# rogeliolopezcamara/prob-matrix-factorization

Measured on AMD Instinct MI355X. Metric: ratings/sec (epoch) Gaussian-MF K=64, higher is better.
Workload: dtype f32; 1 GPU; gaussian_mf_cavi_bias K=64, 1Mx100k synthetic, 50M ratings; n_items=100000, ratings_total=50000000, n_factors=64, ratings_on_rank0=50000000, users_on_rank0=1000000, parallelism=single GPU, torch_imported=False

## Files before the change

prob-matrix-factorization_amd/csrc/pmf_ctx.hip:

```cpp
#include <limits.h>
#include <stdarg.h>
#include <stdlib.h>
#include <stdio.h>
#include <string.h>

#include <algorithm>
#include <exception>
#include <new>

#include "pmf_internal.h"

static thread_local char g_err[512] = "";

void pmf_set_error(const char *fmt, ...) {
    va_list ap;
    va_start(ap, fmt);
    vsnprintf(g_err, sizeof(g_err), fmt, ap);
    va_end(ap);
}

extern "C" const char *pmf_last_error(void) { return g_err; }
extern "C" int pmf_abi_version(void) { return PMF_ABI_VERSION; }

extern "C" int pmf_device_count(int *count) {
// ... 130 lines not shown
    ctx->dtype = dtype;
    ctx->elem = dtype == PMF_F64 ? 8 : 4;
    ctx->rows[0] = n_users;
    ctx->rows[1] = n_items;
    ctx->K = n_factors;
    ctx->kpad = (n_factors + PMF_VEC - 1) / PMF_VEC * PMF_VEC;
    {
        const int line = 128 / (int)ctx->elem;
        if ((ctx->kpad % line) * (int)ctx->elem > 64) ctx->kpad = (ctx->kpad + line - 1) / line * line;
    }
    ctx->kp = n_factors * (n_factors + 1) / 2;
    ctx->cov_stride = (ctx->kp + PMF_VEC - 1) / PMF_VEC * PMF_VEC;
    hipError_t e = hipStreamCreateWithFlags(&ctx->own_stream.s, hipStreamNonBlocking);
    if (e != hipSuccess) {
        pmf_set_error("hipStreamCreate failed: %s", hipGetErrorString(e));
        delete ctx;
        return PMF_EHIP;
    }
    ctx->stream = ctx->own_stream.s;
    ctx->gauss_generic = getenv("PMF_GAUSS_GENERIC") != nullptr;
    ctx->gauss_unfused = getenv("PMF_GAUSS_UNFUSED") != nullptr;
    ctx->gauss_lds_solve = getenv("PMF_GAUSS_LDS_SOLVE") != nullptr;
    ctx->gauss_bias_gather = getenv("PMF_GAUSS_BIAS_GATHER") != nullptr;
    const char *hot_mb = getenv("PMF_GAUSS_HOT_MB");
    ctx->gauss_hot_bytes = (hot_mb ? std::max(atoll(hot_mb), 0LL) : (long long)PMF_GAUSS_HOT_MB_DEFAULT) << 20;
    ctx->topk_two_phase = getenv("PMF_TOPK_TWO_PHASE") != nullptr;
    if (const char *nb = getenv("PMF_TOPK_STAGE_BUFFERS")) ctx->topk_stage_buffers = atoi(nb);
    if (const char *mb = getenv("PMF_TOPK_MAX_BLOCKS")) ctx->topk_max_blocks = atoi(mb);
    if (const char *rt = getenv("PMF_RANK_TARGETS")) ctx->rank_targets = std::max(atoi(rt), 0);
    if (const char *tc = getenv("PMF_TASK_CHUNK")) {
        const int n = atoi(tc);
        if (n >= 32 && n <= 512 && (n & (n - 1)) == 0) ctx->task_chunk = n;
    }
    if (const char *fr = getenv("PMF_FOLD_IN_ROWS")) ctx->fold_in_rows = std::max(atoll(fr), 0LL);
    if (const char *fl = getenv("PMF_GAMMA_FOLD_LONG")) ctx->gamma_fold_long = std::max(atoll(fl), 0LL);
    if (const char *er = getenv("PMF_ELBO_ROWS")) ctx->elbo_rows = std::max(atoll(er), 0LL);
    if (const char *pp = getenv("PMF_GAMMA_PRED_PAIRS")) ctx->gamma_pred_pairs = std::max(atoll(pp), 0LL);
    if (const char *qr = getenv("PMF_TOPK_QUERY_ROWS")) {
        const long long n = atoll(qr);
        ctx->topk_query_rows = n > 0 ? std::max(n / 32 * 32, 32LL) : 0;
    }
    if (const char *sb = getenv("PMF_STAGE_BYTES")) {
        const long long n = atoll(sb);
        if (n > 0) ctx->stage_bytes = n;
    }
    if (const char *ex = getenv("PMF_COMM_EXCHANGE")) {
        if (!strcmp(ex, "allreduce")) ctx->exchange = PMF_EXCHANGE_ALLREDUCE;
        else if (!strcmp(ex, "scatter_gather")) ctx->exchange = PMF_EXCHANGE_SCATTER_GATHER;
    }
    *out = ctx;
    return PMF_OK;
}

static void drop_ratings(pmf_ctx *ctx) {
    pmf_factor_written(ctx);
    ctx->index[0] = PmfSideIndex();
    ctx->index[1] = PmfSideIndex();
    ctx->nnz = 0;
}

struct RatingsGuard {
    pmf_ctx *ctx;
    int finish(int rc) {
        if (rc == PMF_OK) ctx = nullptr;
        return rc;
    }
// ... 111 lines not shown
        for (size_t k = 0; k < raw.size(); ++k) {
            while (raw[k].row >= row_bounds[g + 1]) ++g;
            group[k] = (int32_t)g;
            bucket[g * span + (size_t)(chunk - raw[k].len) + 1]++;
        }
    }
    for (size_t b = 1; b < bucket.size(); ++b) bucket[b] += bucket[b - 1];
    task_off.resize(n_groups + 1);
    for (size_t g = 0; g <= n_groups; ++g) task_off[g] = bucket[g * span];
    tasks.resize(raw.size());
    for (size_t k = 0; k < raw.size(); ++k)
        tasks[(size_t)bucket[(size_t)group[k] * span + (size_t)(chunk - raw[k].len)]++] = raw[k];
    split_off.assign(n_groups + 1, (int64_t)split.size());
    {
        size_t k = 0;
        for (size_t g = 0; g < n_groups; ++g) {
            while (k < split.size() && split[k].row < row_bounds[g]) ++k;
            split_off[g] = (int64_t)k;
        }
    }
}

static std::vector<int64_t> chunk_bounds(const pmf_ctx *ctx, int side) {
    std::vector<int64_t> b((size_t)ctx->n_chunks[side] + 1);
    for (int c = 0; c <= ctx->n_chunks[side]; ++c) b[(size_t)c] = pmf_chunk_row0(ctx, side, c);
    return b;
}

PmfTaskView pmf_task_view(const pmf_ctx *ctx, int side, const PmfTaskList &tl, bool select) {
    const PmfSideIndex &ix = ctx->index[side];
    const int c = select ? ctx->cur_chunk[side] : -1;
    PmfTaskView v;
    v.n_slots = tl.n_slots;
    auto clip = [&](PmfTaskView &w) {
        if (select && ctx->fin_row0 >= 0) {
            w.row0 = std::max(w.row0, ctx->fin_row0);
            w.row1 = std::max(w.row0, std::min(w.row1, ctx->fin_row1));
        }
    };
    if (c < 0 || tl.task_off.empty()) {
        v.d_tasks = tl.d_tasks.as<PmfTask>();
        v.d_split = tl.d_split.as<PmfSplitRow>();
        v.d_split_rows = tl.d_split_rows.as<int32_t>();
        v.n_tasks = tl.n_tasks;
        v.n_split = tl.n_split;
        v.row0 = 0;
        v.row1 = ctx->rows[side];
        v.d_nonempty = ix.d_nonempty.as<int32_t>();
        v.n_nonempty = ix.n_nonempty;
        clip(v);
        return v;
    }
    const size_t g = (size_t)c;
    v.d_tasks = tl.d_tasks.as<PmfTask>() + tl.task_off[g];
    v.n_tasks = tl.task_off[g + 1] - tl.task_off[g];
    v.d_split = tl.d_split.as<PmfSplitRow>() + tl.split_off[g];
    v.d_split_rows = tl.d_split_rows.as<int32_t>() + tl.split_off[g];
    v.n_split = tl.split_off[g + 1] - tl.split_off[g];
    v.row0 = pmf_chunk_row0(ctx, side, c);
    v.row1 = pmf_chunk_row0(ctx, side, c + 1);
    v.d_nonempty = ix.d_nonempty.as<int32_t>() + ix.nonempty_off[g];
    v.n_nonempty = ix.nonempty_off[g + 1] - ix.nonempty_off[g];
    clip(v);
    return v;
}

int pmf_upload_tasks(pmf_ctx *ctx, const std::vector<int64_t> &ptr, int64_t rows, int chunk, bool keep_empty,
                     const std::vector<int64_t> &row_bounds, bool solve_list, PmfTaskList &out) {
    std::vector<PmfTask> tasks;
    std::vector<PmfSplitRow> split;
    int64_t n_slots = 0;
    pmf_build_tasks(ptr, rows, chunk, keep_empty, row_bounds, tasks, split, n_slots, out.task_off, out.split_off);
    out.n_tasks = (int64_t)tasks.size();
    out.n_split = (int64_t)split.size();
    out.n_slots = n_slots;
    out.max_len = 0;
    for (const PmfTask &t : tasks) out.max_len = std::max(out.max_len, t.len);
    int rc = out.d_tasks.alloc(ctx, tasks.size() * sizeof(PmfTask));
    if (rc) return rc;
    rc = out.d_split.alloc(ctx, split.size() * sizeof(PmfSplitRow));
    if (rc) return rc;
    if (!tasks.empty())
        PMF_HIP_CHECK(hipMemcpy(out.d_tasks.as(), tasks.data(), tasks.size() * sizeof(PmfTask), hipMemcpyHostToDevice));
    if (!split.empty())
        PMF_HIP_CHECK(hipMemcpy(out.d_split.as(), split.data(), split.size() * sizeof(PmfSplitRow), hipMemcpyHostToDevice));
    if (!solve_list) return PMF_OK;
    rc = out.d_split_rows.alloc(ctx, split.size() * sizeof(int32_t));
    if (rc) return rc;
    if (!split.empty()) {
        std::vector<int32_t> ids(split.size());
        for (size_t k = 0; k < split.size(); ++k) ids[k] = split[k].row;
        PMF_HIP_CHECK(hipMemcpy(out.d_split_rows.as(), ids.data(), ids.size() * sizeof(int32_t), hipMemcpyHostToDevice));
    }
    return PMF_OK;
}

int pmf_task_chunk(const pmf_ctx *ctx, int max_chunk) {
    if (ctx->task_chunk) return std::min(ctx->task_chunk, max_chunk);
    int64_t c = 32;
    while (c < max_chunk && c * 65536 < ctx->nnz) c <<= 1;
    return (int)c;
}

static int build_work_lists(pmf_ctx *ctx, int side) {
    PmfSideIndex &ix = ctx->index[side];
    const int64_t rows = ctx->rows[side];
    for (PmfTaskList *t : {&ix.gamma_tasks, &ix.gauss_tasks, &ix.bias_tasks, &ix.sgd_tasks}) *t = PmfTaskList();
    const std::vector<int64_t> bounds = chunk_bounds(ctx, side);
    ix.nonempty_off.assign(bounds.size(), (int64_t)ix.h_nonempty.size());
    for (size_t g = 0; g + 1 < bounds.size(); ++g)
        ix.nonempty_off[g] = std::lower_bound(ix.h_nonempty.begin(), ix.h_nonempty.end(), (int32_t)bounds[g]) -
                             ix.h_nonempty.begin();
    int rc;
    if ((rc = pmf_upload_tasks(ctx, ix.h_ptr, rows, pmf_task_chunk(ctx, PMF_GAMMA_CHUNK), true, bounds, true, ix.gamma_tasks))) return rc;
    if ((rc = pmf_upload_tasks(ctx, ix.h_ptr, rows, pmf_task_chunk(ctx, PMF_GAUSS_CHUNK), false, bounds, true, ix.gauss_tasks))) return rc;
    if ((rc = pmf_upload_tasks(ctx, ix.h_ptr, rows, pmf_task_chunk(ctx, PMF_GAMMA_CHUNK), false, bounds, true, ix.bias_tasks))) return rc;
    if ((rc = pmf_upload_tasks(ctx, ix.h_ptr, rows, PMF_SGD_CHUNK, false, bounds, true, ix.sgd_tasks))) return rc;
    return PMF_OK;
}

__global__ void hot_flags_kernel(const int32_t *other, const uint8_t *hot_rows, uint8_t *flags, int64_t n) {
    for (int64_t i = blockIdx.x * (int64_t)blockDim.x + threadIdx.x; i < n; i += (int64_t)gridDim.x * blockDim.x)
        flags[i] = hot_rows[other[i]];
}

static int build_hot_rows(pmf_ctx *ctx) {
    if (ctx->gauss_hot_bytes <= 0 || ctx->dtype != PMF_F32 || ctx->K > 64 || ctx->nnz == 0) return PMF_OK;
    const int64_t row_bytes = (int64_t)(ctx->cov_stride + ctx->kpad) * (int64_t)sizeof(float);
    for (int side = 0; side < 2; ++side) {
        PmfSideIndex &ix = ctx->index[side];
        const int64_t n = std::min(ctx->gauss_hot_bytes / row_bytes, ix.n_nonempty);
        std::vector<int32_t> ids(ix.h_nonempty);
        auto deg = [&](int32_t r) { return ix.h_ptr[(size_t)r + 1] - ix.h_ptr[(size_t)r]; };
        std::partial_sort(ids.begin(), ids.begin() + n, ids.end(), [&](int32_t a, int32_t b) {
            return deg(a) != deg(b) ? deg(a) > deg(b) : a < b;
        });
        ids.resize((size_t)n);
        ix.h_hot.swap(ids);
    }
    int rc;
    for (int side = 0; side < 2; ++side) {
        PmfSideIndex &ix = ctx->index[side];
        const int other = 1 - side;
        std::vector<uint8_t> mask((size_t)ctx->rows[other], 0);
        for (int32_t r : ctx->index[other].h_hot) mask[(size_t)r] = 1;
        PmfBuf d_mask;
        if ((rc = ix.d_other_hot.alloc(ctx, (size_t)ctx->nnz))) return rc;
        if ((rc = d_mask.alloc(ctx, mask.size()))) return rc;
        PMF_HIP_CHECK(hipMemcpy(d_mask.as(), mask.data(), mask.size(), hipMemcpyHostToDevice));
// ... 487 lines not shown
```

prob-matrix-factorization_amd/csrc/pmf_gauss.hip:

```cpp
#include <stdlib.h>

#include <algorithm>
#include <new>
#include <type_traits>
#include <vector>

#include "pmf_device.h"

typedef float f32x16 __attribute__((ext_vector_type(16)));

template <typename T>
struct GaussParams {
    const PmfTask *tasks;
    int64_t n_tasks;
    const PmfSplitRow *split;
    const int32_t *other;
    const T *val;
    const T *factor_other;
    const T *cov_other;
    const T *bias_self;
    const T *bias_other;
    T *partial;
    T *dst_s;
    int64_t dst_s_stride;
// ... 838 lines not shown
    if (t.slot >= 0) {
        out_s = p.partial + (int64_t)t.slot * (stride + kpad);
        out_w = out_s + stride;
        if constexpr (FUSE) {
            if (p.partial_h && h == 0) {
                float *out_h = p.partial_h + (int64_t)t.slot * kpad;
                if (c < kpad) out_h[c] = hlo;
                if (KB == 64 && 32 + c < kpad) out_h[32 + c] = hhi;
            }
        }
    } else {
        out_s = p.dst_s + (int64_t)t.row * p.dst_s_stride;
        out_w = p.dst_w + (int64_t)t.row * p.dst_w_stride;
    }
#pragma unroll
    for (int s = 0; s < NT; ++s) {
        const int q = lane + 64 * s;
        if (q < chunks) {
            const float4 m = reinterpret_cast<const float4 *>(img)[q];
            float4 o = acc[s];
            o.x += m.x;
            o.y += m.y;
            o.z += m.z;
            o.w += m.w;
            reinterpret_cast<float4 *>(out_s)[q] = o;
        }
    }
    if (h == 0) {
        if (c < kpad) out_w[c] = wlo;
        if (KB == 64 && 32 + c < kpad) out_w[32 + c] = whi;
    }
}

template <typename T>
__global__ __launch_bounds__(256) void gauss_combine_kernel(GaussParams<T> p) {
    constexpr int UN = 8;
    const PmfSplitRow sr = p.split[blockIdx.x];
    const int width = p.cov_stride + p.kpad;
    T *out_s = p.dst_s + (int64_t)sr.row * p.dst_s_stride;
    T *out_w = p.dst_w + (int64_t)sr.row * p.dst_w_stride;
    const int total = width + (p.partial_h ? p.kpad : 0);
    for (int e = threadIdx.x * PMF_VEC; e < total; e += 256 * PMF_VEC) {
        const bool hpart = e >= width;
        const T *base = hpart ? p.partial_h + (int64_t)sr.first_slot * p.kpad + (e - width)
                              : p.partial + (int64_t)sr.first_slot * width + e;
        const int64_t step = hpart ? p.kpad : width;
        Vec4<T> acc = zero4<T>();
        int k = 0;
        for (; k + UN <= sr.n_slots; k += UN) {
            Vec4<T> v[UN];
#pragma unroll
            for (int q = 0; q < UN; ++q) v[q] = load4(base + (int64_t)(k + q) * step);
#pragma unroll
            for (int q = 0; q < UN; ++q)
#pragma unroll
                for (int c = 0; c < PMF_VEC; ++c) acc.v[c] += v[q].v[c];
        }
        for (; k < sr.n_slots; ++k) {
            Vec4<T> v = load4(base + (int64_t)k * step);
#pragma unroll
            for (int c = 0; c < PMF_VEC; ++c) acc.v[c] += v.v[c];
        }
        if (e < p.cov_stride) store4(out_s + e, acc);
        else if (!hpart) store4(out_w + (e - p.cov_stride), acc);
        else store4(p.hsplit + (int64_t)blockIdx.x * p.kpad + (e - width), acc);
    }
}


template <typename T>
__global__ __launch_bounds__(256) void gauss_solve_lds_kernel(SolveParams<T> p, T *scratch) {
    extern __shared__ __align__(16) unsigned char smem_raw[];
    const int K = p.K, ld = K + 1;
    T *lds = reinterpret_cast<T *>(smem_raw);
    T *A = scratch ? scratch + (int64_t)blockIdx.x * K * ld : lds;
    T *g = scratch ? lds : lds + K * ld;
    T *prow = g + K;
    T *pcol = prow + K;
    const int tid = threadIdx.x;
    for (int64_t idx = blockIdx.x; idx < p.n; idx += gridDim.x) {
    const int row = p.rows ? p.rows[idx] : (int)(p.row0 + idx);
    const T *S = p.src_s + (int64_t)row * p.src_s_stride;
    if (!p.rows && S[0] == (T)0) continue;
    __syncthreads();
    for (int e = tid; e < K * K; e += 256) {
        const int i = e / K, j = e % K;
        const int lo = i < j ? i : j, hi = i < j ? j : i;
        T s = S[hi * (hi + 1) / 2 + lo] * p.inv_sigma2;
        if (i == j) s += p.inv_eta2;
        A[i * ld + j] = s;
    }
    __syncthreads();
    for (int i = tid; i < K; i += 256) g[i] = (T)1 / sqrt(A[i * ld + i]);
    __syncthreads();
    for (int e = tid; e < K * K; e += 256) {
        const int i = e / K, j = e % K;
        A[i * ld + j] *= g[i] * g[j];
    }
// ... 119 lines not shown
template <typename T, int LPR>
__global__ __launch_bounds__(256) void gauss_bias_sums_kernel(BiasParams<T> p, const T *mdot) {
    constexpr int G = 256 / LPR;
    constexpr int UN = 4;
    const int c = threadIdx.x % LPR;
    const int64_t task_id = (int64_t)blockIdx.x * G + threadIdx.x / LPR;
    if (task_id >= p.n_tasks) return;
    const PmfTask t = p.tasks[task_id];
    const int32_t *col = p.other + t.start;
    const T *val = p.val + t.start;
    T sum = (T)0;
    for (int base = c; base < t.len; base += UN * LPR) {
        int o[UN];
        T x[UN], b[UN];
#pragma unroll
        for (int q = 0; q < UN; ++q) {
            const int j = min(base + q * LPR, t.len - 1);
            o[q] = col[j];
            x[q] = val[j];
        }
#pragma unroll
        for (int q = 0; q < UN; ++q) b[q] = p.bias_other[o[q]];
#pragma unroll
        for (int q = 0; q < UN; ++q)
            if (base + q * LPR < t.len) sum += x[q] - b[q];
    }
    sum = group_sum<LPR>(sum);
    if (c != 0) return;
    if (t.slot >= 0) p.partial[t.slot] = sum;
    else p.bias_self[t.row] = bias_from_sum(p, sum - mdot[t.row], (T)t.len);
}

template <typename T, bool STATS>
__global__ void gauss_bias_split_kernel(BiasParams<T> p, int64_t n_split, const int64_t *ptr, const T *mdot) {
    const int64_t s = (int64_t)blockIdx.x * blockDim.x + threadIdx.x;
    if (s >= n_split) return;
    const PmfSplitRow sr = p.split[s];
    T sum = (T)0;
    for (int k = 0; k < sr.n_slots; ++k) sum += p.partial[sr.first_slot + k];
    if (mdot) sum -= mdot[sr.row];
    const T cnt = (T)(ptr[sr.row + 1] - ptr[sr.row]);
    if (STATS) {
        p.stats[(int64_t)sr.row * 2] = sum;
        p.stats[(int64_t)sr.row * 2 + 1] = cnt;
    } else {
        p.bias_self[sr.row] = bias_from_sum(p, sum, cnt);
    }
}

template <typename T>
__global__ void gauss_bias_finalize_all_kernel(BiasParams<T> p) {
    const int64_t r = p.row0 + (int64_t)blockIdx.x * blockDim.x + threadIdx.x;
    if (r >= p.rows) return;
    const T cnt = p.stats[r * 2 + 1];
    if (cnt > (T)0) p.bias_self[r] = bias_from_sum(p, p.stats[r * 2], cnt);
}

template <typename T>
struct FoldBiasParams {
    const int64_t *ptr;
    int64_t n;
    const int32_t *other;
    const T *val;
    const T *factor_other;
    const T *bias_other;
    const T *cov;
    T *factor;
    T *bias;
    T inv_sigma2, inv_eta_bias2;
    int n_iter, K, kpad, cov_stride;
};

// ... 191 lines not shown
            pmf_with_pow2<8>(ctx->K, [&](auto KR) {
                hipLaunchKernelGGL((gauss_accum_generic_kernel<T, KR>), grid, dim3(256), lds, ctx->stream, p, is2, ie2, p.dst_s, p.dst_w);
            });
            return true;
        }
    }
    hipLaunchKernelGGL((gauss_accum_generic_kernel<T, 0>), grid, dim3(256), plain, ctx->stream, p, (T)0, (T)0,
                       (T *)nullptr, (T *)nullptr);
    return false;
}

template <typename T>
static GaussParams<T> gauss_params(const pmf_ctx *ctx, int side) {
    const int other = 1 - side;
    const PmfSideIndex &ix = ctx->index[side];
    const bool bias = pmf_has_bias(ctx);
    GaussParams<T> p;
    p.other = ix.d_other.as<int32_t>();
    p.val = ix.d_val.as<const T>();
    p.factor_other = ctx->arr[other][PMF_ARR_FACTOR].as<const T>();
    p.cov_other = ctx->arr[other][PMF_ARR_COV].as<const T>();
    p.hot = ix.d_other_hot.as<uint8_t>();
    p.bias_self = bias ? ctx->arr[side][PMF_ARR_BIAS].as<const T>() : nullptr;
    p.bias_other = bias ? ctx->arr[other][PMF_ARR_BIAS].as<const T>() : nullptr;
    p.partial = ctx->d_partial.as<T>();
    p.K = ctx->K;
    p.kpad = ctx->kpad;
    p.kp = ctx->kp;
    p.cov_stride = ctx->cov_stride;
    return p;
}

template <typename T>
static int launch_accumulate(pmf_ctx *ctx, const GaussParams<T> &p, int64_t n_split, bool fuse = false, double sigma2 = 1,
                             double eta2 = 1, bool *solved = nullptr) {
    bool did = false;
    if (p.n_tasks > 0) {
        PmfProfScope prof(ctx, PMF_KERNEL_GAUSS_ACCUM);
        const T is2 = (T)(1.0 / sigma2), ie2 = (T)(1.0 / eta2);
        if (std::is_same<T, float>::value && !ctx->gauss_generic && ctx->K <= 128) {
            if constexpr (std::is_same<T, float>::value) did = launch_accum_mfma_fp32(ctx, p, fuse, is2, ie2);
        } else {
            did = launch_accum_generic(ctx, p, fuse && ctx->K <= 64, is2, ie2);
        }
    }
    if (solved) *solved = did;
    if (n_split > 0) {
        PmfProfScope prof(ctx, PMF_KERNEL_GAUSS_COMBINE);
        hipLaunchKernelGGL((gauss_combine_kernel<T>), dim3((unsigned)n_split), dim3(256), 0, ctx->stream, p);
    }
    PMF_HIP_CHECK(hipGetLastError());
    return PMF_OK;
}

template <typename T>
static T *gauss_partial_h(const pmf_ctx *ctx, const PmfTaskView &tl) {
    return ctx->d_partial.as<T>() + tl.n_slots * (ctx->cov_stride + ctx->kpad);
}

template <typename T>
static int run_factor_accumulate(pmf_ctx *ctx, int side, PmfPass pass, void *stats, double sigma2, double eta2,
                                 bool *fused = nullptr, bool *sums = nullptr) {
    const int other = 1 - side;
    const PmfSideIndex &ix = ctx->index[side];
    const bool acc = pass == PMF_PASS_ACCUMULATE;
    const PmfTaskView tl = pmf_task_view(ctx, side, ix.gauss_tasks, acc);
    int rc;
    PMF_REQUIRE(ix.d_ptr, PMF_EINVAL, "pmf_gauss_factor_sweep: ratings have not been set");
    if ((rc = pmf_require_array(ctx, side, PMF_ARR_FACTOR, "pmf_gauss_factor_sweep"))) return rc;
    if ((rc = pmf_require_array(ctx, side, PMF_ARR_COV, "pmf_gauss_factor_sweep"))) return rc;
    if ((rc = pmf_require_array(ctx, other, PMF_ARR_FACTOR, "pmf_gauss_factor_sweep"))) return rc;
    if ((rc = pmf_require_array(ctx, other, PMF_ARR_COV, "pmf_gauss_factor_sweep"))) return rc;
    const int width = ctx->cov_stride + ctx->kpad;
    const bool fuse = !acc && !ctx->gauss_unfused;
    const bool emit = sums && fuse && std::is_same<T, float>::value && !ctx->gauss_generic && ctx->K <= 64 &&
                      !ctx->gauss_bias_gather && pmf_has_bias(ctx) && !pmf_comm_active(ctx);
    const size_t h_elems = emit ? (size_t)(tl.n_slots + tl.n_split) * ctx->kpad : 0;
    if (tl.n_slots > 0 && (rc = pmf_ensure_partial(ctx, ((size_t)tl.n_slots * width + h_elems) * sizeof(T)))) return rc;
    if (emit && (rc = ctx->d_mdot[side].reserve(ctx, (size_t)ctx->rows[side] * sizeof(T), {ctx->stream}))) return rc;
    if (acc && tl.row1 > tl.row0)
        PMF_HIP_CHECK(hipMemsetAsync((T *)stats + tl.row0 * width, 0, (size_t)(tl.row1 - tl.row0) * width * sizeof(T), ctx->stream));
    GaussParams<T> p = gauss_params<T>(ctx, side);
    p.tasks = tl.d_tasks;
    p.n_tasks = tl.n_tasks;
    p.split = tl.d_split;
    if (emit) {
        p.mdot = ctx->d_mdot[side].as<T>();
        p.partial_h = gauss_partial_h<T>(ctx, tl);
        p.hsplit = p.partial_h + tl.n_slots * ctx->kpad;
    }
    if (sums) *sums = emit;
    p.dst_s = acc ? (T *)stats : ctx->arr[side][PMF_ARR_COV].as<T>();
    p.dst_s_stride = acc ? width : ctx->cov_stride;
    p.dst_w = acc ? (T *)stats + ctx->cov_stride : ctx->arr[side][PMF_ARR_FACTOR].as<T>();
    p.dst_w_stride = acc ? width : ctx->kpad;
    return launch_accumulate<T>(ctx, p, tl.n_split, fuse, sigma2, eta2, fused);
}

template <typename T>
static int launch_solve(pmf_ctx *ctx, const SolveParams<T> &sp) {
    int rc;
    if (sp.n == 0) return PMF_OK;
    PmfProfScope prof(ctx, PMF_KERNEL_GAUSS_SOLVE);
    if (ctx->K <= 64)
        pmf_with_pow2<8>(ctx->K, [&](auto KR) {
            hipLaunchKernelGGL((gauss_solve_reg_kernel<T, KR>), dim3((unsigned)((sp.n + 3) / 4)), dim3(256),
                               (size_t)4 * ctx->cov_stride * sizeof(T), ctx->stream, sp);
        });
    else if (std::is_same<T, float>::value && !ctx->gauss_lds_solve && ctx->K <= 128) {
        if constexpr (std::is_same<T, float>::value) {
            const size_t smem = (size_t)PAIR_LDS_FLOATS * sizeof(float);
            switch ((ctx->K + 15) / 16) {
                case 5: hipLaunchKernelGGL((gauss_solve_pair_kernel<5>), dim3((unsigned)sp.n), dim3(128), smem, ctx->stream, sp); break;
                case 6: hipLaunchKernelGGL((gauss_solve_pair_kernel<6>), dim3((unsigned)sp.n), dim3(128), smem, ctx->stream, sp); break;
                case 7: hipLaunchKernelGGL((gauss_solve_pair_kernel<7>), dim3((unsigned)sp.n), dim3(128), smem, ctx->stream, sp); break;
                default: hipLaunchKernelGGL((gauss_solve_pair_kernel<8>), dim3((unsigned)sp.n), dim3(128), smem, ctx->stream, sp); break;
            }
        }
    } else {
        const int K = ctx->K;
        const size_t mat = (size_t)K * (K + 1) * sizeof(T), vecs = (size_t)3 * K * sizeof(T);
        const bool in_lds = mat + vecs <= (size_t)160 * 1024;
        const unsigned blocks = (unsigned)std::min<int64_t>(sp.n, in_lds ? sp.n : 2048);
        T *scratch = nullptr;
        if (!in_lds) {
            if ((rc = pmf_ensure_scratch(ctx, (size_t)blocks * mat))) return rc;
            scratch = ctx->d_scratch.as<T>();
        }
        const size_t smem = in_lds ? mat + vecs : vecs;
// ... 101 lines not shown
    p.factor_other = ctx->arr[other][PMF_ARR_FACTOR].as<const T>();
    p.bias_self = ctx->arr[side][PMF_ARR_BIAS].as<T>();
    p.bias_other = ctx->arr[other][PMF_ARR_BIAS].as<const T>();
    p.partial = ctx->d_partial.as<T>();
    p.stats = (T *)stats;
    p.inv_sigma2 = acc ? (T)1 : (T)(1.0 / sigma2);
    p.inv_eta_bias2 = acc ? (T)1 : (T)(1.0 / eta_bias2);
    p.kpad = ctx->kpad;
    p.row0 = tl.row0;
    p.rows = tl.row1;
    const bool from_sums = pass == PMF_PASS_FUSED && std::is_same<T, float>::value && ctx->gauss_mdot_valid[side] &&
                           !ctx->gauss_bias_gather && !pmf_comm_active(ctx);
    const T *mdot = from_sums ? ctx->d_mdot[side].as<const T>() : nullptr;
    PmfProfScope prof(ctx, PMF_KERNEL_GAUSS_BIAS);
    if (pass == PMF_PASS_FINALIZE) {
        if (p.rows > p.row0)
            hipLaunchKernelGGL((gauss_bias_finalize_all_kernel<T>), dim3((unsigned)((p.rows - p.row0 + 255) / 256)), dim3(256), 0,
                               ctx->stream, p);
    } else {
        if (acc && p.rows > p.row0)
            PMF_HIP_CHECK(hipMemsetAsync((T *)stats + p.row0 * 2, 0, (size_t)(p.rows - p.row0) * 2 * sizeof(T), ctx->stream));
        if (tl.n_tasks > 0 && from_sums) {
            if (ctx->nnz / tl.n_tasks >= 64)
                hipLaunchKernelGGL((gauss_bias_sums_kernel<T, 64>), dim3((unsigned)((p.n_tasks + 3) / 4)), dim3(256), 0, ctx->stream, p, mdot);
            else
                hipLaunchKernelGGL((gauss_bias_sums_kernel<T, 16>), dim3((unsigned)((p.n_tasks + 15) / 16)), dim3(256), 0, ctx->stream, p, mdot);
        } else if (tl.n_tasks > 0)
            pmf_with_pow2<1>(pmf_lanes_per_row(ctx->kpad), [&](auto L) {
                dim3 grid((unsigned)((p.n_tasks + 256 / L - 1) / (256 / L)));
                if (acc) hipLaunchKernelGGL((gauss_bias_kernel<T, L, true>), grid, dim3(256), 0, ctx->stream, p);
                else hipLaunchKernelGGL((gauss_bias_kernel<T, L, false>), grid, dim3(256), 0, ctx->stream, p);
            });
        if (tl.n_split > 0) {
            dim3 grid((unsigned)((tl.n_split + 255) / 256));
            if (acc) hipLaunchKernelGGL((gauss_bias_split_kernel<T, true>), grid, dim3(256), 0, ctx->stream, p, tl.n_split, ix.d_ptr.as<int64_t>(), mdot);
            else hipLaunchKernelGGL((gauss_bias_split_kernel<T, false>), grid, dim3(256), 0, ctx->stream, p, tl.n_split, ix.d_ptr.as<int64_t>(), mdot);
        }
    }
    PMF_HIP_CHECK(hipGetLastError());
    return PMF_OK;
}

extern "C" int pmf_gauss_bias_sweep(pmf_ctx *ctx, int side, double sigma2, double eta_bias2) {
    PMF_SIDE_ENTRY("pmf_gauss_bias_sweep");
    return pmf_with_dtype(ctx, [&](auto t) {
        using T = decltype(t);
        if (side != PMF_SIDE_ITEM || !pmf_comm_active(ctx)) return run_bias<T>(ctx, side, PMF_PASS_FUSED, nullptr, sigma2, eta_bias2);
        const PmfExchange ex = {false, 1, {PMF_ARR_BIAS}};
        return pmf_comm_half_sweep(ctx, side, 1, 2, false, ex,
                                   [&](void *s) { return run_bias<T>(ctx, side, PMF_PASS_ACCUMULATE, s, 1, 1); },
                                   [&](void *s) { return run_bias<T>(ctx, side, PMF_PASS_FINALIZE, s, sigma2, eta_bias2); });
    });
}

extern "C" int pmf_gauss_bias_accumulate(pmf_ctx *ctx, int side, void *stats_dev) {
    PMF_SIDE_ENTRY("pmf_gauss_bias_accumulate");
    PMF_REQUIRE(stats_dev, PMF_EINVAL, "pmf_gauss_bias_accumulate: null stats buffer");
    return pmf_with_dtype(ctx, [&](auto t) { return run_bias<decltype(t)>(ctx, side, PMF_PASS_ACCUMULATE, stats_dev, 1, 1); });
}

extern "C" int pmf_gauss_bias_finalize(pmf_ctx *ctx, int side, const void *stats_dev, double sigma2,
                                       double eta_bias2) {
    PMF_SIDE_ENTRY("pmf_gauss_bias_finalize");
    PMF_REQUIRE(stats_dev, PMF_EINVAL, "pmf_gauss_bias_finalize: null stats buffer");
    return pmf_with_dtype(ctx, [&](auto t) { return run_bias<decltype(t)>(ctx, side, PMF_PASS_FINALIZE, (void *)stats_dev, sigma2, eta_bias2); });
}

// ... 45 lines not shown
        if ((rc = d_split.reserve(ctx, split.size() * sizeof(PmfSplitRow), {ctx->stream}))) return rc;
        if ((rc = d_ptr.reserve(ctx, ptr.size() * sizeof(int64_t), {ctx->stream}))) return rc;
        if ((rc = d_other.reserve(ctx, (size_t)nnz * sizeof(int32_t), {ctx->stream}))) return rc;
        if ((rc = d_val.reserve(ctx, (size_t)nnz * sizeof(T), {ctx->stream}))) return rc;
        if ((rc = d_s.reserve(ctx, (size_t)B * cs * sizeof(T), {ctx->stream}))) return rc;
        if ((rc = d_w.reserve(ctx, (size_t)B * kpad * sizeof(T), {ctx->stream}))) return rc;
        if ((rc = d_b.reserve(ctx, (size_t)B * sizeof(T), {ctx->stream}))) return rc;
        if ((rc = d_partial.reserve(ctx, (size_t)n_slots * width * sizeof(T), {ctx->stream}))) return rc;
        PMF_HIP_CHECK(hipMemcpy(d_ptr.as(), ptr.data(), ptr.size() * sizeof(int64_t), hipMemcpyHostToDevice));
        if (nnz) {
            PMF_HIP_CHECK(hipMemcpy(d_tasks.as(), tasks.data(), tasks.size() * sizeof(PmfTask), hipMemcpyHostToDevice));
            PMF_HIP_CHECK(hipMemcpy(d_other.as(), a.other_ids + at, (size_t)nnz * sizeof(int32_t), hipMemcpyHostToDevice));
            PMF_HIP_CHECK(hipMemcpy(d_val.as(), val.data(), (size_t)nnz * sizeof(T), hipMemcpyHostToDevice));
        }
        if (!split.empty())
            PMF_HIP_CHECK(hipMemcpy(d_split.as(), split.data(), split.size() * sizeof(PmfSplitRow), hipMemcpyHostToDevice));
        if (has_empty) {
            PMF_HIP_CHECK(hipMemsetAsync(d_s.as(), 0, (size_t)B * cs * sizeof(T), ctx->stream));
            PMF_HIP_CHECK(hipMemsetAsync(d_w.as(), 0, (size_t)B * kpad * sizeof(T), ctx->stream));
        }
        GaussParams<T> p = gauss_params<T>(ctx, side);
        p.tasks = d_tasks.as<PmfTask>();
        p.n_tasks = (int64_t)tasks.size();
        p.split = d_split.as<PmfSplitRow>();
        p.other = d_other.as<int32_t>();
        p.val = d_val.as<const T>();
        p.hot = nullptr;
        p.bias_self = nullptr;
        p.partial = d_partial.as<T>();
        p.dst_s = d_s.as<T>();
        p.dst_s_stride = cs;
        p.dst_w = d_w.as<T>();
        p.dst_w_stride = kpad;
        if ((rc = launch_accumulate<T>(ctx, p, (int64_t)split.size()))) return rc;
        SolveParams<T> sp = solve_params<T>(ctx, a.sigma2, a.eta2);
        sp.rows = nullptr;
        sp.row0 = 0;
        sp.n = B;
        sp.src_s = d_s.as<const T>();
        sp.src_s_stride = cs;
        sp.src_w = d_w.as<const T>();
        sp.src_w_stride = kpad;
        sp.cov = d_s.as<T>();
        sp.factor = d_w.as<T>();
        if ((rc = launch_solve<T>(ctx, sp))) return rc;
        if (bias) {
            FoldBiasParams<T> q;
            q.ptr = d_ptr.as<const int64_t>();
            q.n = B;
            q.other = p.other;
            q.val = p.val;
            q.factor_other = p.factor_other;
            q.bias_other = p.bias_other;
            q.cov = d_s.as<const T>();
            q.factor = d_w.as<T>();
            q.bias = d_b.as<T>();
            q.inv_sigma2 = (T)(1.0 / a.sigma2);
            q.inv_eta_bias2 = (T)(1.0 / a.eta_bias2);
            q.n_iter = a.n_iter;
            q.K = K;
            q.kpad = kpad;
            q.cov_stride = cs;
            PmfProfScope prof(ctx, PMF_KERNEL_GAUSS_BIAS);
            pmf_with_pow2<1>(pmf_lanes_per_row(kpad), [&](auto L) {
                dim3 grid((unsigned)((B + 256 / L - 1) / (256 / L)));
                hipLaunchKernelGGL((gauss_fold_bias_kernel<T, L>), grid, dim3(256), 0, ctx->stream, q);
            });
// ... 369 lines not shown
    e.bias = bias ? ctx->arr[side][PMF_ARR_BIAS].as<const T>() : nullptr;
    e.out = d_out.as<double>();
    e.K = ctx->K;
    e.kpad = kpad;
    e.kp = ctx->kp;
    e.cov_stride = cs;
    if (!with_data) {
        e.row0 = 0;
        e.n = rows;
        PmfProfScope prof(ctx, PMF_KERNEL_GAUSS_SOLVE);
        if ((rc = launch_elbo_rows<T>(ctx, e))) return rc;
    } else {
        const int64_t win_rows = std::min(elbo_window_rows<T>(ctx), rows);
        if ((rc = ensure_elbo_tasks(ctx, side, win_rows))) return rc;
        const PmfTaskList &tl = ix.elbo_tasks;
        if (tl.n_slots > 0 && (rc = pmf_ensure_partial(ctx, (size_t)tl.n_slots * width * sizeof(T)))) return rc;
        if ((rc = d_cpart.alloc(ctx, (size_t)tl.n_slots * sizeof(T)))) return rc;
        if ((rc = d_win.alloc(ctx, (size_t)win_rows * width * sizeof(T)))) return rc;
        if ((rc = d_c.alloc(ctx, (size_t)win_rows * sizeof(T)))) return rc;
        GaussParams<T> p = gauss_params<T>(ctx, side);
        p.dst_s_stride = width;
        p.dst_w_stride = width;
        e.stats = d_win.as<const T>();
        e.csum = d_c.as<const T>();
        e.ptr = ix.d_ptr.as<const int64_t>();
        for (size_t w = 0; w + 1 < ix.elbo_bounds.size(); ++w) {
            const int64_t r0 = ix.elbo_bounds[w], n = ix.elbo_bounds[w + 1] - r0;
            const int64_t nt = tl.task_off[w + 1] - tl.task_off[w], ns = tl.split_off[w + 1] - tl.split_off[w];
            p.tasks = tl.d_tasks.as<PmfTask>() + tl.task_off[w];
            p.n_tasks = nt;
            p.split = tl.d_split.as<PmfSplitRow>() + tl.split_off[w];
            p.dst_s = reinterpret_cast<T *>(reinterpret_cast<uintptr_t>(d_win.as<T>()) - (uintptr_t)r0 * width * sizeof(T));
            p.dst_w = p.dst_s + cs;
            if ((rc = launch_accumulate<T>(ctx, p, ns))) return rc;
            PmfProfScope prof(ctx, PMF_KERNEL_GAUSS_SOLVE);
            if (nt > 0) {
                ElboSqParams<T> q;
                q.tasks = p.tasks;
                q.n_tasks = nt;
                q.other = p.other;
                q.val = p.val;
                q.bias_self = p.bias_self;
                q.bias_other = p.bias_other;
                q.partial = d_cpart.as<T>();
                q.csum = d_c.as<T>();
                q.row0 = r0;
                hipLaunchKernelGGL((gauss_elbo_sq_kernel<T>), dim3((unsigned)((nt + 15) / 16)), dim3(256), 0, ctx->stream, q);
            }
            if (ns > 0)
                hipLaunchKernelGGL((gauss_elbo_sq_split_kernel<T>), dim3((unsigned)((ns + 255) / 256)), dim3(256), 0, ctx->stream,
                                   p.split, ns, d_cpart.as<const T>(), d_c.as<T>(), r0);
            PMF_HIP_CHECK(hipGetLastError());
            e.row0 = r0;
            e.n = n;
            if ((rc = launch_elbo_rows<T>(ctx, e))) return rc;
        }
    }
    std::vector<double> host;
    double *dst = per_row;
    if (!dst) {
        host.resize((size_t)rows * PMF_ELBO_TERMS);
        dst = host.data();
    }
    PMF_HIP_CHECK(hipMemcpyAsync(dst, d_out.as(), (size_t)rows * PMF_ELBO_TERMS * sizeof(double), hipMemcpyDeviceToHost,
                                 ctx->stream));
    PMF_HIP_CHECK(hipStreamSynchronize(ctx->stream));
    double sum[PMF_ELBO_TERMS] = {};
// ... 22 lines not shown
```

prob-matrix-factorization_amd/csrc/pmf_internal.h:

```cpp
#pragma once

#include <hip/hip_runtime.h>
#include <stdint.h>

#include <functional>
#include <initializer_list>
#include <new>
#include <string>
#include <type_traits>
#include <utility>
#include <vector>

#include "pmf_hip.h"

#ifndef PMF_TRANSPORT_HOSTSHM
#define PMF_TRANSPORT_HOSTSHM 1
#endif

#define PMF_WAVE 64
#define PMF_VEC 4
#define PMF_RATE_FLOOR 1e-10
#define PMF_MAX_LABELS 32

void pmf_set_error(const char *fmt, ...);
// ... 51 lines not shown
    int reserve(pmf_ctx *owner, size_t bytes, std::initializer_list<hipStream_t> sync);
    void reset();
    template <typename T = void>
    T *as() const { return static_cast<T *>(p_); }
    explicit operator bool() const { return p_ != nullptr; }

private:
    void *p_ = nullptr;
    size_t bytes_ = 0;
    pmf_ctx *owner_ = nullptr;
    bool pinned_;
};

struct PmfTask {
    int64_t start;
    int32_t row;
    int32_t len;
    int32_t slot;
    int32_t pad;
};

struct PmfSplitRow {
    int32_t row;
    int32_t first_slot;
    int32_t n_slots;
    int32_t pad;
};

struct PmfTaskList {
    int64_t n_tasks = 0;
    int64_t n_slots = 0;
    int64_t n_split = 0;
    int32_t max_len = 0;
    PmfBuf d_tasks;
    PmfBuf d_split;
    PmfBuf d_split_rows;
    std::vector<int64_t> task_off, split_off;
};

struct PmfTaskView {
    const PmfTask *d_tasks = nullptr;
    const PmfSplitRow *d_split = nullptr;
    const int32_t *d_split_rows = nullptr;
    int64_t n_tasks = 0, n_split = 0, n_slots = 0;
    int64_t row0 = 0, row1 = 0;
    const int32_t *d_nonempty = nullptr;
    int64_t n_nonempty = 0;
};

struct PmfSideIndex {
    PmfBuf d_ptr;
    PmfBuf d_other;
    PmfBuf d_val;
    std::vector<int64_t> h_ptr;
    PmfBuf d_nonempty;
    int64_t n_nonempty = 0;
    std::vector<int32_t> h_nonempty;
    std::vector<int64_t> nonempty_off;
    PmfTaskList gamma_tasks;
    PmfTaskList gauss_tasks;
    PmfTaskList bias_tasks;
    PmfTaskList sgd_tasks;
    PmfTaskList elbo_tasks;
    std::vector<int64_t> elbo_bounds;
    PmfBuf d_distinct_ptr;
    PmfBuf d_distinct;
    std::vector<int32_t> h_hot;
    PmfBuf d_other_hot;
};

struct PmfEvalSet {
    int64_t n = 0;
    int n_labels = 0;
    PmfBuf d_u, d_i;
    PmfBuf d_y;
    PmfBuf d_label;
};
// ... 19 lines not shown

    int n_chunks[2] = {1, 1};
    int cur_chunk[2] = {-1, -1};
    int64_t fin_row0 = -1, fin_row1 = -1;
    int exchange = PMF_EXCHANGE_AUTO;

    PmfBuf arr[2][PMF_ARR_COUNT];
    PmfSideIndex index[2];
    PmfEvalSet eval;

    PmfBuf d_partial, d_scratch;
    PmfBuf d_mdot[2];
    bool gauss_mdot_valid[2] = {false, false};
    PmfBuf d_gamma_tables;
    PmfBuf h_pinned{PmfBuf::PINNED};

    bool gauss_generic = false;
    bool gauss_unfused = false;
    bool gauss_lds_solve = false;
    bool gauss_bias_gather = false;
    int64_t gauss_hot_bytes = 0;
    int topk_max_blocks = 0;
    int topk_stage_buffers = 0;
    bool topk_two_phase = false;
    int rank_targets = 0;
    int64_t fold_in_rows = 0;
    int64_t gamma_fold_long = 0;
    int64_t gamma_pred_pairs = 0;
    int64_t topk_query_rows = 0;
    int64_t stage_bytes = 64ll << 20;
    int64_t elbo_rows = 0;
    size_t elbo_lds_bytes = 0;
    int task_chunk = 0;

    struct PmfComm *comm = nullptr;
    PmfBuf d_stats[2];

    bool prof = false;
    struct ProfRec {
        hipEvent_t a, b;
        int kernel;
    };
    std::vector<ProfRec> prof_pending;
    std::vector<hipEvent_t> prof_pool;
    double prof_ms[PMF_KERNEL_COUNT] = {};
    int64_t prof_n[PMF_KERNEL_COUNT] = {};

    ~pmf_ctx();
};

#define PMF_GAMMA_CHUNK 512
#define PMF_SGD_CHUNK 256
#define PMF_GAUSS_CHUNK 512
#define PMF_FOLD_IN_BLOCK_NNZ (32ll << 20)
#define PMF_GAUSS_HOT_MB_DEFAULT 224

static inline int64_t pmf_chunk_row0(const pmf_ctx *ctx, int side, int c) {
    return ctx->rows[side] * (int64_t)c / ctx->n_chunks[side];
}
void pmf_build_tasks(const std::vector<int64_t> &ptr, int64_t rows, int chunk, bool keep_empty,
                     const std::vector<int64_t> &row_bounds, std::vector<PmfTask> &tasks, std::vector<PmfSplitRow> &split,
                     int64_t &n_slots, std::vector<int64_t> &task_off, std::vector<int64_t> &split_off);
int pmf_upload_tasks(pmf_ctx *ctx, const std::vector<int64_t> &ptr, int64_t rows, int chunk, bool keep_empty,
                     const std::vector<int64_t> &row_bounds, bool solve_list, PmfTaskList &out);
int pmf_task_chunk(const pmf_ctx *ctx, int max_chunk);
PmfTaskView pmf_task_view(const pmf_ctx *ctx, int side, const PmfTaskList &tl, bool select);

int pmf_ensure_partial(pmf_ctx *ctx, size_t bytes);
int pmf_ensure_scratch(pmf_ctx *ctx, size_t bytes);
int pmf_ensure_pinned(pmf_ctx *ctx, size_t bytes);
int pmf_allow_dynamic_lds(const void *kernel, size_t bytes);
size_t pmf_array_elems(const pmf_ctx *ctx, int side, int array);
int pmf_require_array(pmf_ctx *ctx, int side, int array, const char *what);
int pmf_alloc_array(pmf_ctx *ctx, int side, int array);

struct PmfIndexBuild;
int pmf_index_device_begin(pmf_ctx *ctx, int64_t nnz, const int32_t *user_ids, const int32_t *item_ids,
                           const double *ratings, PmfIndexBuild **out, int64_t *bad_position);
void pmf_index_device_abort(PmfIndexBuild *b);
int pmf_index_device_finish(pmf_ctx *ctx, PmfIndexBuild *b, int64_t nnz);
int pmf_index_distinct(pmf_ctx *ctx, int side);

void pmf_array_shape(const pmf_ctx *ctx, int array, int *host_width, int *dev_stride);
void pmf_unpack_rows(const pmf_ctx *ctx, int array, const void *src, double *dst, int64_t rows);
int pmf_fold_in_download(pmf_ctx *ctx, int array, const void *dev, double *host, int64_t rows);

bool pmf_comm_active(const pmf_ctx *ctx);
void pmf_comm_release(pmf_ctx *ctx);
int pmf_comm_wait_stream(pmf_ctx *ctx, hipStream_t stream, const char *what);
struct PmfExchange {
    bool prefer_scatter = false;
    int n_arrays = 0;
    int arrays[6] = {0, 0, 0, 0, 0, 0};
};
int pmf_comm_half_sweep(pmf_ctx *ctx, int side, int which, size_t width, bool chunked, const PmfExchange &ex,
                        const std::function<int(void *)> &accumulate, const std::function<int(void *)> &finalize);

void pmf_prof_begin(pmf_ctx *ctx, int kernel);
// ... 40 lines not shown
```

Measured before the change: 420.2 million ratings/s.

## Raise Gauss task chunk and parallelise split-row combine hierarchically

The maximum task chunk for the Gaussian and bias sweeps rises to 1024 and gains its own environment override. With nnz=50M the default heuristic now picks 1024 instead of 512, so there are fewer tasks. The split-row combine becomes two levels: groups of 32 slots are summed in parallel over a second grid dimension, then a second launch sums the group results. The bias split kernel now uses a 64-lane wavefront per row with a group reduction instead of one thread per row. These changes aim to cut per-task overhead and the serial reduction cost of heavy rows, at the price of an extra kernel launch and changed work sizes.

```diff
diff --git a/prob-matrix-factorization_amd/csrc/pmf_ctx.hip b/prob-matrix-factorization_amd/csrc/pmf_ctx.hip
--- a/prob-matrix-factorization_amd/csrc/pmf_ctx.hip
+++ b/prob-matrix-factorization_amd/csrc/pmf_ctx.hip
@@ -186,6 +186,10 @@
         const int n = atoi(tc);
         if (n >= 32 && n <= 512 && (n & (n - 1)) == 0) ctx->task_chunk = n;
     }
+    if (const char *gc = getenv("PMF_GAUSS_TASK_CHUNK")) {
+        const int n = atoi(gc);
+        if (n >= 32 && n <= PMF_GAUSS_SWEEP_CHUNK_MAX && (n & (n - 1)) == 0) ctx->gauss_task_chunk = n;
+    }
     if (const char *fr = getenv("PMF_FOLD_IN_ROWS")) ctx->fold_in_rows = std::max(atoll(fr), 0LL);
     if (const char *fl = getenv("PMF_GAMMA_FOLD_LONG")) ctx->gamma_fold_long = std::max(atoll(fl), 0LL);
     if (const char *er = getenv("PMF_ELBO_ROWS")) ctx->elbo_rows = std::max(atoll(er), 0LL);
@@ -363,6 +367,7 @@
     const int c = select ? ctx->cur_chunk[side] : -1;
     PmfTaskView v;
     v.n_slots = tl.n_slots;
+    v.max_row_slots = tl.max_row_slots;
     auto clip = [&](PmfTaskView &w) {
         if (select && ctx->fin_row0 >= 0) {
             w.row0 = std::max(w.row0, ctx->fin_row0);
@@ -407,6 +412,8 @@
     out.n_slots = n_slots;
     out.max_len = 0;
     for (const PmfTask &t : tasks) out.max_len = std::max(out.max_len, t.len);
+    out.max_row_slots = 0;
+    for (const PmfSplitRow &r : split) out.max_row_slots = std::max(out.max_row_slots, r.n_slots);
     int rc = out.d_tasks.alloc(ctx, tasks.size() * sizeof(PmfTask));
     if (rc) return rc;
     rc = out.d_split.alloc(ctx, split.size() * sizeof(PmfSplitRow));
@@ -433,6 +440,11 @@
     return (int)c;
 }
 
+int pmf_gauss_sweep_chunk(const pmf_ctx *ctx) {
+    if (ctx->gauss_task_chunk) return ctx->gauss_task_chunk;
+    return pmf_task_chunk(ctx, PMF_GAUSS_SWEEP_CHUNK_MAX);
+}
+
 static int build_work_lists(pmf_ctx *ctx, int side) {
     PmfSideIndex &ix = ctx->index[side];
     const int64_t rows = ctx->rows[side];
@@ -444,8 +456,8 @@
                              ix.h_nonempty.begin();
     int rc;
     if ((rc = pmf_upload_tasks(ctx, ix.h_ptr, rows, pmf_task_chunk(ctx, PMF_GAMMA_CHUNK), true, bounds, true, ix.gamma_tasks))) return rc;
-    if ((rc = pmf_upload_tasks(ctx, ix.h_ptr, rows, pmf_task_chunk(ctx, PMF_GAUSS_CHUNK), false, bounds, true, ix.gauss_tasks))) return rc;
-    if ((rc = pmf_upload_tasks(ctx, ix.h_ptr, rows, pmf_task_chunk(ctx, PMF_GAMMA_CHUNK), false, bounds, true, ix.bias_tasks))) return rc;
+    if ((rc = pmf_upload_tasks(ctx, ix.h_ptr, rows, pmf_gauss_sweep_chunk(ctx), false, bounds, true, ix.gauss_tasks))) return rc;
+    if ((rc = pmf_upload_tasks(ctx, ix.h_ptr, rows, pmf_gauss_sweep_chunk(ctx), false, bounds, true, ix.bias_tasks))) return rc;
     if ((rc = pmf_upload_tasks(ctx, ix.h_ptr, rows, PMF_SGD_CHUNK, false, bounds, true, ix.sgd_tasks))) return rc;
     return PMF_OK;
 }
diff --git a/prob-matrix-factorization_amd/csrc/pmf_gauss.hip b/prob-matrix-factorization_amd/csrc/pmf_gauss.hip
--- a/prob-matrix-factorization_amd/csrc/pmf_gauss.hip
+++ b/prob-matrix-factorization_amd/csrc/pmf_gauss.hip
@@ -894,38 +894,49 @@
     }
 }
 
-template <typename T>
-__global__ __launch_bounds__(256) void gauss_combine_kernel(GaussParams<T> p) {
-    constexpr int UN = 8;
+#define PMF_COMBINE_GROUP 32
+template <typename T>
+__global__ __launch_bounds__(256) void gauss_combine_kernel(GaussParams<T> p, int level) {
+    constexpr int UN = 8, G = PMF_COMBINE_GROUP;
     const PmfSplitRow sr = p.split[blockIdx.x];
+    const bool grouped = sr.n_slots > G;
+    if (level == 1 && !grouped) return;
     const int width = p.cov_stride + p.kpad;
     T *out_s = p.dst_s + (int64_t)sr.row * p.dst_s_stride;
     T *out_w = p.dst_w + (int64_t)sr.row * p.dst_w_stride;
     const int total = width + (p.partial_h ? p.kpad : 0);
-    for (int e = threadIdx.x * PMF_VEC; e < total; e += 256 * PMF_VEC) {
-        const bool hpart = e >= width;
-        const T *base = hpart ? p.partial_h + (int64_t)sr.first_slot * p.kpad + (e - width)
-                              : p.partial + (int64_t)sr.first_slot * width + e;
-        const int64_t step = hpart ? p.kpad : width;
-        Vec4<T> acc = zero4<T>();
-        int k = 0;
-        for (; k + UN <= sr.n_slots; k += UN) {
-            Vec4<T> v[UN];
-#pragma unroll
-            for (int q = 0; q < UN; ++q) v[q] = load4(base + (int64_t)(k + q) * step);
-#pragma unroll
-            for (int q = 0; q < UN; ++q)
-#pragma unroll
-                for (int c = 0; c < PMF_VEC; ++c) acc.v[c] += v[q].v[c];
-        }
-        for (; k < sr.n_slots; ++k) {
-            Vec4<T> v = load4(base + (int64_t)k * step);
-#pragma unroll
-            for (int c = 0; c < PMF_VEC; ++c) acc.v[c] += v.v[c];
-        }
-        if (e < p.cov_stride) store4(out_s + e, acc);
-        else if (!hpart) store4(out_w + (e - p.cov_stride), acc);
-        else store4(p.hsplit + (int64_t)blockIdx.x * p.kpad + (e - width), acc);
+    const int n_groups = (sr.n_slots + G - 1) / G;
+    const int stride = level == 1 ? G : 1;
+    for (int g = level == 1 ? 0 : (int)blockIdx.y; g < (level == 1 ? 1 : n_groups); g += (int)gridDim.y) {
+        const int first = level == 1 ? 0 : g * G;
+        const int n = level == 1 ? n_groups : min(G, sr.n_slots - first);
+        const bool to_slot = level == 0 && grouped;
+        for (int e = threadIdx.x * PMF_VEC; e < total; e += 256 * PMF_VEC) {
+            const bool hpart = e >= width;
+            T *base = hpart ? p.partial_h + (int64_t)(sr.first_slot + first) * p.kpad + (e - width)
+                            : p.partial + (int64_t)(sr.first_slot + first) * width + e;
+            const int64_t step = (int64_t)stride * (hpart ? p.kpad : width);
+            Vec4<T> acc = zero4<T>();
+            int k = 0;
+            for (; k + UN <= n; k += UN) {
+                Vec4<T> v[UN];
+#pragma unroll
+                for (int q = 0; q < UN; ++q) v[q] = load4(base + (int64_t)(k + q) * step);
+#pragma unroll
+                for (int q = 0; q < UN; ++q)
+#pragma unroll
+                    for (int c = 0; c < PMF_VEC; ++c) acc.v[c] += v[q].v[c];
+            }
+            for (; k < n; ++k) {
+                Vec4<T> v = load4(base + (int64_t)k * step);
+#pragma unroll
+                for (int c = 0; c < PMF_VEC; ++c) acc.v[c] += v.v[c];
+            }
+            if (to_slot) store4(base, acc);
+            else if (e < p.cov_stride) store4(out_s + e, acc);
+            else if (!hpart) store4(out_w + (e - p.cov_stride), acc);
+            else store4(p.hsplit + (int64_t)blockIdx.x * p.kpad + (e - width), acc);
+        }
     }
 }
 
@@ -1111,12 +1122,15 @@
 }
 
 template <typename T, bool STATS>
-__global__ void gauss_bias_split_kernel(BiasParams<T> p, int64_t n_split, const int64_t *ptr, const T *mdot) {
-    const int64_t s = (int64_t)blockIdx.x * blockDim.x + threadIdx.x;
+__global__ __launch_bounds__(256) void gauss_bias_split_kernel(BiasParams<T> p, int64_t n_split, const int64_t *ptr, const T *mdot) {
+    const int c = threadIdx.x % 64;
+    const int64_t s = (int64_t)blockIdx.x * 4 + threadIdx.x / 64;
     if (s >= n_split) return;
     const PmfSplitRow sr = p.split[s];
     T sum = (T)0;
-    for (int k = 0; k < sr.n_slots; ++k) sum += p.partial[sr.first_slot + k];
+    for (int k = c; k < sr.n_slots; k += 64) sum += p.partial[sr.first_slot + k];
+    sum = group_sum<64>(sum);
+    if (c != 0) return;
     if (mdot) sum -= mdot[sr.row];
     const T cnt = (T)(ptr[sr.row + 1] - ptr[sr.row]);
     if (STATS) {
@@ -1374,8 +1388,8 @@
 }
 
 template <typename T>
-static int launch_accumulate(pmf_ctx *ctx, const GaussParams<T> &p, int64_t n_split, bool fuse = false, double sigma2 = 1,
-                             double eta2 = 1, bool *solved = nullptr) {
+static int launch_accumulate(pmf_ctx *ctx, const GaussParams<T> &p, int64_t n_split, int max_row_slots, bool fuse = false,
+                             double sigma2 = 1, double eta2 = 1, bool *solved = nullptr) {
     bool did = false;
     if (p.n_tasks > 0) {
         PmfProfScope prof(ctx, PMF_KERNEL_GAUSS_ACCUM);
@@ -1389,7 +1403,10 @@
     if (solved) *solved = did;
     if (n_split > 0) {
         PmfProfScope prof(ctx, PMF_KERNEL_GAUSS_COMBINE);
-        hipLaunchKernelGGL((gauss_combine_kernel<T>), dim3((unsigned)n_split), dim3(256), 0, ctx->stream, p);
+        const int groups = (max_row_slots + PMF_COMBINE_GROUP - 1) / PMF_COMBINE_GROUP;
+        const dim3 grid((unsigned)n_split, (unsigned)std::min(std::max(groups, 1), 8));
+        hipLaunchKernelGGL((gauss_combine_kernel<T>), grid, dim3(256), 0, ctx->stream, p, 0);
+        if (groups > 1) hipLaunchKernelGGL((gauss_combine_kernel<T>), dim3((unsigned)n_split), dim3(256), 0, ctx->stream, p, 1);
     }
     PMF_HIP_CHECK(hipGetLastError());
     return PMF_OK;
@@ -1436,7 +1453,7 @@
     p.dst_s_stride = acc ? width : ctx->cov_stride;
     p.dst_w = acc ? (T *)stats + ctx->cov_stride : ctx->arr[side][PMF_ARR_FACTOR].as<T>();
     p.dst_w_stride = acc ? width : ctx->kpad;
-    return launch_accumulate<T>(ctx, p, tl.n_split, fuse, sigma2, eta2, fused);
+    return launch_accumulate<T>(ctx, p, tl.n_split, tl.max_row_slots, fuse, sigma2, eta2, fused);
 }
 
 template <typename T>
@@ -1604,7 +1621,7 @@
                 else hipLaunchKernelGGL((gauss_bias_kernel<T, L, false>), grid, dim3(256), 0, ctx->stream, p);
             });
         if (tl.n_split > 0) {
-            dim3 grid((unsigned)((tl.n_split + 255) / 256));
+            dim3 grid((unsigned)((tl.n_split + 3) / 4));
             if (acc) hipLaunchKernelGGL((gauss_bias_split_kernel<T, true>), grid, dim3(256), 0, ctx->stream, p, tl.n_split, ix.d_ptr.as<int64_t>(), mdot);
             else hipLaunchKernelGGL((gauss_bias_split_kernel<T, false>), grid, dim3(256), 0, ctx->stream, p, tl.n_split, ix.d_ptr.as<int64_t>(), mdot);
         }
@@ -1716,7 +1733,9 @@
         p.dst_s_stride = cs;
         p.dst_w = d_w.as<T>();
         p.dst_w_stride = kpad;
-        if ((rc = launch_accumulate<T>(ctx, p, (int64_t)split.size()))) return rc;
+        int max_row_slots = 0;
+        for (const PmfSplitRow &sr : split) max_row_slots = std::max(max_row_slots, sr.n_slots);
+        if ((rc = launch_accumulate<T>(ctx, p, (int64_t)split.size(), max_row_slots))) return rc;
         SolveParams<T> sp = solve_params<T>(ctx, a.sigma2, a.eta2);
         sp.rows = nullptr;
         sp.row0 = 0;
@@ -2152,7 +2171,7 @@
             p.split = tl.d_split.as<PmfSplitRow>() + tl.split_off[w];
             p.dst_s = reinterpret_cast<T *>(reinterpret_cast<uintptr_t>(d_win.as<T>()) - (uintptr_t)r0 * width * sizeof(T));
             p.dst_w = p.dst_s + cs;
-            if ((rc = launch_accumulate<T>(ctx, p, ns))) return rc;
+            if ((rc = launch_accumulate<T>(ctx, p, ns, tl.max_row_slots))) return rc;
             PmfProfScope prof(ctx, PMF_KERNEL_GAUSS_SOLVE);
             if (nt > 0) {
                 ElboSqParams<T> q;
diff --git a/prob-matrix-factorization_amd/csrc/pmf_internal.h b/prob-matrix-factorization_amd/csrc/pmf_internal.h
--- a/prob-matrix-factorization_amd/csrc/pmf_internal.h
+++ b/prob-matrix-factorization_amd/csrc/pmf_internal.h
@@ -107,6 +107,7 @@
     int64_t n_slots = 0;
     int64_t n_split = 0;
     int32_t max_len = 0;
+    int32_t max_row_slots = 0;
     PmfBuf d_tasks;
     PmfBuf d_split;
     PmfBuf d_split_rows;
@@ -118,6 +119,7 @@
     const PmfSplitRow *d_split = nullptr;
     const int32_t *d_split_rows = nullptr;
     int64_t n_tasks = 0, n_split = 0, n_slots = 0;
+    int32_t max_row_slots = 0;
     int64_t row0 = 0, row1 = 0;
     const int32_t *d_nonempty = nullptr;
     int64_t n_nonempty = 0;
@@ -203,6 +205,7 @@
     int64_t elbo_rows = 0;
     size_t elbo_lds_bytes = 0;
     int task_chunk = 0;
+    int gauss_task_chunk = 0;
 
     struct PmfComm *comm = nullptr;
     PmfBuf d_stats[2];
@@ -223,6 +226,7 @@
 #define PMF_GAMMA_CHUNK 512
 #define PMF_SGD_CHUNK 256
 #define PMF_GAUSS_CHUNK 512
+#define PMF_GAUSS_SWEEP_CHUNK_MAX 1024
 #define PMF_FOLD_IN_BLOCK_NNZ (32ll << 20)
 #define PMF_GAUSS_HOT_MB_DEFAULT 224
 
@@ -235,6 +239,7 @@
 int pmf_upload_tasks(pmf_ctx *ctx, const std::vector<int64_t> &ptr, int64_t rows, int chunk, bool keep_empty,
                      const std::vector<int64_t> &row_bounds, bool solve_list, PmfTaskList &out);
 int pmf_task_chunk(const pmf_ctx *ctx, int max_chunk);
+int pmf_gauss_sweep_chunk(const pmf_ctx *ctx);
 PmfTaskView pmf_task_view(const pmf_ctx *ctx, int side, const PmfTaskList &tl, bool select);
 
 int pmf_ensure_partial(pmf_ctx *ctx, size_t bytes);
```

New measurement: 421.3 million ratings/s (median of 2 runs). About the same (+0.3%).
